# tomer-erez/Psychoacoustic-adverserial-attacks

Hardware: AMD Instinct MI355X
Metric: pgd_steps_per_sec (higher is better)
Workload: dtype bf16x3 (split-bf16 hi+lo, three MFMA passes, f32 accumulate: fp32-parity); 1 GPU; untargeted PGD, norm_type snr snr_db 40, Wav2Vec2-base (rule-generated weights), 32x10s 16 kHz clips per GPU, 150-token labels; global_batch=32, per_gpu_batch=32, samples_per_clip=160000, parallelism=dp1, hip_graph=True, hip_graph_replayed_steps=80

## Files before the change

psychoacoustic-adverserial-attacks_amd/csrc/gemm.hip:

```cpp
#include <algorithm>
#include <vector>

#include "gemm_dev.h"

namespace paa {

template <int ROWS, bool IS_A>
__device__ __forceinline__ void load_kc(const paa_gemm_desc& d, const float* __restrict__ base, int64_t ld, int r0,
                                        int k0, int rlim, float4 (&v)[ROWS / 32]) {
    const int tid = threadIdx.x;
    const int k = k0 + ((tid & 7) << 2);
    int64_t koff = k;
    int js = 0, kc = k;
    if (IS_A && d.a_kseg > 0) {
        js = k / d.a_kseg;
        kc = k - js * d.a_kseg;
        koff = (int64_t)js * d.a_kseg_stride + kc;
    }
#pragma unroll
    for (int i = 0; i < ROWS / 32; ++i) {
        const int r = r0 + (tid >> 3) + 32 * i;
        float4 x = make_float4(0.f, 0.f, 0.f, 0.f);
        bool ok = (r < rlim) && (k < d.K);
        const float* p;
// ... 536 lines not shown

static int g_ring_mode = 0;
struct GemmEnv { bool init = false, no_sq = false, no_r2 = false, kgroup = true, no_bil = false; };
static GemmEnv g_env;
static void gemm_env_refresh() {
#ifdef PAA_EXPERIMENTS
    auto on = [](const char* name, char v) { const char* e = getenv(name); return e && e[0] == v; };
    g_env.no_sq = on("PAA_NO_SQ", '1');
    g_env.no_r2 = on("PAA_NO_R2", '1');
    g_env.kgroup = !on("PAA_K_GROUP", '0');
    g_env.no_bil = on("PAA_NO_BIL", '1');
#endif
    g_env.init = true;
}
bool gemm_env_no_bil() {
    if (!g_env.init) gemm_env_refresh();
    return g_env.no_bil;
}
bool gemm_env_kgroup() {
    if (!g_env.init) gemm_env_refresh();
    return g_env.kgroup;
}

static int g_last_kind = EPK_GENERIC;
static int classify_epilogue(const paa_gemm_desc& d) {
#ifdef PAA_EXPERIMENTS
    { const char* e = getenv("PAA_NO_EPIK"); if (e && e[0] == '1') return EPK_GENERIC; }
#endif
    if (d.alpha != 1.f || d.accumulate || d.aux_bf16 || !d.precision) return EPK_GENERIC;
    const bool il = d.Cb_il && !d.Cb && !d.Cb_lo, planar = d.Cb && d.Cb_lo && !d.Cb_il, no_planes = !d.Cb && !d.Cb_lo && !d.Cb_il;
    const bool mask = d.row_period > 0;
    switch (d.act) {
        case PAA_ACT_GELU:
            return (d.bias && d.C_pre && d.aux_gate && il && !d.C && !d.aux && !d.residual && !d.res_ln_stats) ? EPK_GELU_FWD : EPK_GENERIC;
        case PAA_ACT_GELU_GRAD:
            if (!(d.aux && d.aux_gate && (il || planar) && !d.bias && !d.C && !d.C_pre && !d.residual && !d.res_ln_stats && !mask)) return EPK_GENERIC;
#ifdef PAA_EXPERIMENTS
            { const char* e = getenv("PAA_EPIK_AHEAD"); if (e && e[0] == '2') return EPK_GELU_GRAD_LA2; if (e && e[0] == '4') return EPK_GELU_GRAD_LA4; }
#endif
            return EPK_GELU_GRAD;
        case PAA_ACT_NONE:
            if (d.C_pre || d.aux || d.aux_gate || mask) return EPK_GENERIC;
            if (d.C && no_planes && d.residual) {
                if (d.res_ln_stats) return d.bias ? EPK_RESID_LN : EPK_GENERIC;
                return d.bias ? EPK_GENERIC : EPK_RESID;
            }
            if (!d.C && planar && !d.residual && !d.res_ln_stats) return EPK_PLANES;
            return EPK_GENERIC;
        default: return EPK_GENERIC;
    }
}

template <int BN, int PREC>
static void launch_gemm(const GemmArgs& g, dim3 grid, hipStream_t st) {
    const bool akc = g.d.a_kcontig != 0, bkc = g.d.b_kcontig != 0;
    if (akc && bkc) hipLaunchKernelGGL((k_gemm<BN, PREC, true, true>), grid, dim3(G_NT), 0, st, g);
    else if (akc && !bkc) hipLaunchKernelGGL((k_gemm<BN, PREC, true, false>), grid, dim3(G_NT), 0, st, g);
    else if (!akc && bkc) hipLaunchKernelGGL((k_gemm<BN, PREC, false, true>), grid, dim3(G_NT), 0, st, g);
    else hipLaunchKernelGGL((k_gemm<BN, PREC, false, false>), grid, dim3(G_NT), 0, st, g);
}

struct GemmProf {
    bool on = false;
    std::vector<hipEvent_t> ev;
    std::vector<double> flops, bytes;
    std::vector<int> variant;
    size_t n = 0, cap = 0;
};
static GemmProf g_prof;

paa_status gemm(const paa_gemm_desc& d, hipStream_t st) {
// ... 120 lines not shown
        d.ldb >= d.K && d.a_kseg_stride == d.lda) {
        const int taps = d.K / d.a_kseg;
        const int npl = d.precision ? 2 : 1;
        const int mi = (d.a_kseg == 48 && d.M > 128) ? 2 : 1;
        const size_t lds = 2 * (size_t)npl * ((size_t)(128 * mi + taps - 1) * (d.a_kseg + 8) + 64 * (size_t)(4 * d.a_kseg + 8));
        if (lds <= 150 * 1024) {
            dim3 wgrid(cdiv(d.M, 128 * mi), d.batch);
#define PAA_WIN(P, KS_, MI_, WV_)                                                                                            \
            {                                                                                                                \
                static bool attr = false;                                                                                    \
                if (!attr) { PAA_HIP(hipFuncSetAttribute(reinterpret_cast<const void*>(&k_gemm_win<P, KS_, MI_, WV_>), hipFuncAttributeMaxDynamicSharedMemorySize, 152 * 1024)); attr = true; } \
                hipLaunchKernelGGL((k_gemm_win<P, KS_, MI_, WV_>), wgrid, dim3(WV_ * 64), lds, st, g, taps);                 \
            }
            if (prof) { g_prof.variant[g_prof.n] = 40 + (d.precision ? 4 : 0); }
            if (d.a_kseg == 48) {
                if (mi == 2) { if (d.precision) PAA_WIN(1, 48, 1, 8) else PAA_WIN(0, 48, 2, 4) }
                else { if (d.precision) PAA_WIN(1, 48, 1, 4) else PAA_WIN(0, 48, 1, 4) }
            }
            else { if (d.precision) PAA_WIN(1, 64, 1, 4) else PAA_WIN(0, 64, 1, 4) }
#undef PAA_WIN
            if (prof) { (void)hipEventRecord(g_prof.ev[2 * g_prof.n + 1], st); ++g_prof.n; }
            PAA_LAUNCH_CHECK();
            return PAA_OK;
        }
    }
    if (ring) {
        if (prof) g_prof.variant[g_prof.n] = (ring_bm == 192 ? (ring_bn == 128 ? 60 : 52) : (ring_bn == 256 ? 56 : 48)) + (d.precision ? 1 : 0);
#ifdef PAA_EXPERIMENTS
        if (ring == 13) launch_bf<192, 128, 1, 2, true, false, true>(g, st);
        else
#endif
        if (ring >= 20) {
            g.kind = g_last_kind = classify_epilogue(d);
            int taken = 1 << EPK_GELU_FWD;
#ifdef PAA_EXPERIMENTS
            { const char* e = getenv("PAA_EPIK_MASK"); const int mask = e ? atoi(e) : 0; if (mask > 0) taken = mask; }
#endif
            if (!((taken >> g.kind) & 1)) g.kind = EPK_GENERIC;
            launch_ring2_cfg(ring, g, st);
        }
        else launch_ring_cfg(ring, g, st);
    } else if (d.operand_bf16) {
        const bool seg = d.a_kseg > 0 || (d.K & 63);
        if (narrow) {
            if (seg) { if (d.precision) launch_bf<128, 64, 1, 2, false, true>(g, st); else launch_bf<128, 64, 0, 2, false, true>(g, st); }
            else { if (d.precision) launch_bf<128, 64, 1, 2, false, false>(g, st); else launch_bf<128, 64, 0, 2, false, false>(g, st); }
        }
        else if (seg && vec && !d.precision) launch_bf<128, 128, 0, 2, true, true>(g, st);
        else if (seg) { if (d.precision) launch_bf<128, 128, 1, 2, false, true>(g, st); else launch_bf<128, 128, 0, 2, false, true>(g, st); }
        else if (tall) {
            if (d.precision) launch_bf<256, 128, 1, 4, true, false>(g, st);
            else if (bm192) launch_bf<192, 128, 0, 2, true, false>(g, st);
            else launch_bf<256, 128, 0, 2, true, false>(g, st);
        }
        else if (vec) { if (d.precision) launch_bf<128, 128, 1, 2, true, false>(g, st); else launch_bf<128, 128, 0, 2, true, false>(g, st); }
        else { if (d.precision) launch_bf<128, 128, 1, 2, false, false>(g, st); else launch_bf<128, 128, 0, 2, false, false>(g, st); }
    } else if (narrow) { if (d.precision) launch_gemm<64, 1>(g, grid, st); else launch_gemm<64, 0>(g, grid, st); }
    else { if (d.precision) launch_gemm<128, 1>(g, grid, st); else launch_gemm<128, 0>(g, grid, st); }
    if (prof) { (void)hipEventRecord(g_prof.ev[2 * g_prof.n + 1], st); ++g_prof.n; }
    PAA_LAUNCH_CHECK();
    return PAA_OK;
}

}

extern "C" paa_status paa_prof_enable(int max_launches) {
    using namespace paa;
// ... 44 lines not shown
```

psychoacoustic-adverserial-attacks_amd/csrc/gemm_dev.h:

```cpp
#pragma once
#include "gemm.h"
#include "paa_common.h"

namespace paa {

typedef short bf16x8 __attribute__((ext_vector_type(8)));
typedef float f32x16 __attribute__((ext_vector_type(16)));

constexpr int G_BM = 128, G_BK = 32, G_LD = 40 , G_NT = 256;


struct GemmArgs {
    paa_gemm_desc d;
    int tiles_m, tiles_n;
    int kind;
};

enum { EPK_GENERIC = 0, EPK_GELU_FWD = 1, EPK_GELU_GRAD = 2, EPK_RESID = 3, EPK_RESID_LN = 4, EPK_PLANES = 5,
       EPK_GELU_GRAD_LA2 = 6, EPK_GELU_GRAD_LA4 = 7, EPK_COUNT = 8 };
enum { EPI_NO = 0, EPI_YES = 1, EPI_RT = 2 };
template <int S>
__device__ __forceinline__ bool epi_on(bool rt) {
    if constexpr (S == EPI_RT) return rt;
    else return S == EPI_YES;
}
struct EpiGeneric {
    static constexpr int ACT = -1, BIAS = EPI_RT, C = EPI_RT, CPRE = EPI_RT, X16 = EPI_RT, GATE = EPI_RT, CIL = EPI_RT, CB = EPI_RT, CBLO = EPI_RT,
                         RES = EPI_RT, RLN = EPI_RT, PERIOD = EPI_RT, ACCUM = EPI_RT;
    static constexpr bool ALPHA1 = false;
    static constexpr int AHEAD = 1;
};
struct EpiGeluFwd {
    static constexpr int ACT = PAA_ACT_GELU, BIAS = EPI_YES, C = EPI_NO, CPRE = EPI_YES, X16 = EPI_NO, GATE = EPI_YES, CIL = EPI_YES, CB = EPI_NO, CBLO = EPI_NO,
                         RES = EPI_NO, RLN = EPI_NO, PERIOD = EPI_RT, ACCUM = EPI_NO;
    static constexpr bool ALPHA1 = true;
    static constexpr int AHEAD = 1;
};
struct EpiGeluGrad {
    static constexpr int ACT = PAA_ACT_GELU_GRAD, BIAS = EPI_NO, C = EPI_NO, CPRE = EPI_NO, X16 = EPI_NO, GATE = EPI_YES, CIL = EPI_RT, CB = EPI_YES, CBLO = EPI_YES,
                         RES = EPI_NO, RLN = EPI_NO, PERIOD = EPI_NO, ACCUM = EPI_NO;
    static constexpr bool ALPHA1 = true;
    static constexpr int AHEAD = 1;
};
template <int AH>
struct EpiGeluGradAhead : EpiGeluGrad {
    static constexpr int AHEAD = AH;
};
struct EpiResid {
    static constexpr int ACT = PAA_ACT_NONE, BIAS = EPI_NO, C = EPI_YES, CPRE = EPI_NO, X16 = EPI_NO, GATE = EPI_NO, CIL = EPI_NO, CB = EPI_NO, CBLO = EPI_NO,
                         RES = EPI_YES, RLN = EPI_NO, PERIOD = EPI_NO, ACCUM = EPI_NO;
    static constexpr bool ALPHA1 = true;
    static constexpr int AHEAD = 1;
};
struct EpiResidLn {
    static constexpr int ACT = PAA_ACT_NONE, BIAS = EPI_YES, C = EPI_YES, CPRE = EPI_NO, X16 = EPI_NO, GATE = EPI_NO, CIL = EPI_NO, CB = EPI_NO, CBLO = EPI_NO,
                         RES = EPI_YES, RLN = EPI_YES, PERIOD = EPI_NO, ACCUM = EPI_NO;
    static constexpr bool ALPHA1 = true;
    static constexpr int AHEAD = 1;
};
struct EpiPlanes {
    static constexpr int ACT = PAA_ACT_NONE, BIAS = EPI_RT, C = EPI_NO, CPRE = EPI_NO, X16 = EPI_NO, GATE = EPI_NO, CIL = EPI_NO, CB = EPI_YES, CBLO = EPI_YES,
                         RES = EPI_NO, RLN = EPI_NO, PERIOD = EPI_NO, ACCUM = EPI_NO;
    static constexpr bool ALPHA1 = true;
    static constexpr int AHEAD = 1;
};

template <typename K>
inline int blocks_per_cu(K kernel, int threads) {
    int per = 0;
    if (hipOccupancyMaxActiveBlocksPerMultiprocessor(&per, kernel, threads, 0) != hipSuccess) return 0;
    return per;
}

template <int NJ, int MI>
__device__ __forceinline__ void epilogue(const paa_gemm_desc& d, f32x16 (&acc)[MI][NJ], int mw, int nw, int z1, int z2) {
    const int64_t coff = z1 * d.c_s1 + z2 * d.c_s2 + (int64_t)mw * d.ldc + nw;
    float* __restrict__ C = d.C ? d.C + coff : nullptr;
    const bool x16 = d.aux_bf16 != 0;
    float* __restrict__ Cp = (d.C_pre && !x16) ? d.C_pre + coff : nullptr;
    unsigned short* __restrict__ Cp16 = (d.C_pre && x16) ? reinterpret_cast<unsigned short*>(d.C_pre) + coff : nullptr;
    unsigned short* __restrict__ Cb = d.Cb ? reinterpret_cast<unsigned short*>(d.Cb) + coff : nullptr;
    unsigned short* __restrict__ Cbl = d.Cb_lo ? reinterpret_cast<unsigned short*>(d.Cb_lo) + coff : nullptr;
    unsigned short* __restrict__ Cil = d.Cb_il ? reinterpret_cast<unsigned short*>(d.Cb_il) + 2 * (z1 * d.c_s1 + z2 * d.c_s2) : nullptr;
    const int64_t xoff = z1 * d.aux_s1 + z2 * d.aux_s2 + (int64_t)mw * d.ld_aux + nw;
    const float* __restrict__ aux = (d.aux && !x16) ? d.aux + xoff : nullptr;
    const unsigned short* __restrict__ aux16 = (d.aux && x16) ? reinterpret_cast<const unsigned short*>(d.aux) + xoff : nullptr;
    const float* __restrict__ res = d.residual ? d.residual + z1 * d.res_s1 + z2 * d.res_s2 + (int64_t)mw * d.ld_res + nw : nullptr;
    const float* __restrict__ bias = d.bias ? d.bias + z2 * d.bias_s2 + nw : nullptr;
    const int ldc = (int)d.ldc, ld_aux = (int)d.ld_aux, ld_res = (int)d.ld_res;
    const int period = d.row_period;
    const int mrem0 = period > 0 ? mw % period : 0;
    const int act = d.act;
    const float alpha = d.alpha;
#pragma unroll
    for (int i = 0; i < MI; ++i) {
        const int64_t ro = (int64_t)(i * 32) * ldc;
        float* __restrict__ Ci = C ? C + ro : nullptr;
// ... 55 lines not shown
                    Cbi[ci] = h;
                    if (Cbli) Cbli[ci] = bf16_bits(v - bf16_to_f32(h));
                }
                if (Cil) {
                    const int n = nw + dn;
                    const int64_t o = (int64_t)(mw + i * 32 + dm) * (2 * d.ldc) + ((n >> 5) << 6) + (n & 31);
                    const unsigned short h = bf16_bits(v);
                    Cil[o] = h;
                    Cil[o + 32] = bf16_bits(v - bf16_to_f32(h));
                }
            }
        }
    }
}

__device__ __forceinline__ float dpp_quad_xor1(float v) {
    return __int_as_float(__builtin_amdgcn_mov_dpp(__float_as_int(v), 0xB1, 0xF, 0xF, true));
}
__device__ __forceinline__ float dpp_quad_xor2(float v) {
    return __int_as_float(__builtin_amdgcn_mov_dpp(__float_as_int(v), 0x4E, 0xF, 0xF, true));
}
__device__ __forceinline__ void quad_transpose(float& x0, float& x1, float& x2, float& x3, bool o1, bool o2) {
    float s = dpp_quad_xor1(o1 ? x0 : x1);
    float t = dpp_quad_xor1(o1 ? x2 : x3);
    if (o1) { x0 = s; x2 = t; } else { x1 = s; x3 = t; }
    s = dpp_quad_xor2(o2 ? x0 : x2);
    t = dpp_quad_xor2(o2 ? x1 : x3);
    if (o2) { x0 = s; x1 = t; } else { x2 = s; x3 = t; }
}

__device__ __forceinline__ float mul_unfused(float a, float b) {
#pragma clang fp contract(off)
    return a * b;
}

template <int MI, bool FAST, typename T = EpiGeneric>
__device__ __forceinline__ void epilogue_vec(const paa_gemm_desc& d, f32x16 (&acc)[MI][2], int m0w, int n0w, int z1, int z2, int lane) {
    const int lr = lane & 31, lh = lane >> 5, qa = lr >> 2, qb = lr & 3;
    const bool o1 = qb & 1, o2 = qb & 2;
    const int col = n0w + 8 * qa;
    const int row0 = m0w + 4 * lh + qb;
    const bool col_ok = col < d.N;
    const int act = T::ACT < 0 ? d.act : T::ACT;
    const bool gg = act == PAA_ACT_GELU_GRAD;
    const int64_t cbase = z1 * d.c_s1 + z2 * d.c_s2;
    float* __restrict__ C = epi_on<T::C>(d.C != nullptr) ? d.C + cbase : nullptr;
    const bool has_c = T::C == EPI_RT ? C != nullptr : T::C == EPI_YES;
    const bool x16 = epi_on<T::X16>(d.aux_bf16 != 0);
    const bool gate = epi_on<T::GATE>(d.aux_gate != 0);
    float* __restrict__ Cp = (epi_on<T::CPRE>(d.C_pre != nullptr) && !x16) ? d.C_pre + cbase : nullptr;
    unsigned short* __restrict__ Cp16 = (epi_on<T::CPRE>(d.C_pre != nullptr) && x16) ? reinterpret_cast<unsigned short*>(d.C_pre) + cbase : nullptr;
    constexpr bool PRE_RT = T::CPRE == EPI_RT || T::X16 == EPI_RT;
    const bool has_cp = PRE_RT ? Cp != nullptr : (T::CPRE == EPI_YES && T::X16 == EPI_NO);
    const bool has_cp16 = PRE_RT ? Cp16 != nullptr : (T::CPRE == EPI_YES && T::X16 == EPI_YES);
    unsigned short* __restrict__ Cb = epi_on<T::CB>(d.Cb != nullptr) ? reinterpret_cast<unsigned short*>(d.Cb) + cbase : nullptr;
    unsigned short* __restrict__ Cbl = epi_on<T::CBLO>(d.Cb_lo != nullptr) ? reinterpret_cast<unsigned short*>(d.Cb_lo) + cbase : nullptr;
    const bool cil = epi_on<T::CIL>(d.Cb_il != nullptr);
    if (cil) { Cb = reinterpret_cast<unsigned short*>(d.Cb_il) + 2 * cbase; Cbl = Cb + 32; }
    const bool has_cb = (T::CIL == EPI_YES || T::CB == EPI_YES) ? true : (T::CIL == EPI_NO && T::CB == EPI_NO) ? false : Cb != nullptr;
    const bool has_cbl = (T::CIL == EPI_YES || T::CBLO == EPI_YES) ? true : (T::CIL == EPI_NO && T::CBLO == EPI_NO) ? false : Cbl != nullptr;
    const bool ex16 = gg && x16;
    const float* __restrict__ ex = gg ? (ex16 ? nullptr : d.aux + z1 * d.aux_s1 + z2 * d.aux_s2)
                                      : (epi_on<T::RES>(d.residual != nullptr) ? d.residual + z1 * d.res_s1 + z2 * d.res_s2 : nullptr);
    const unsigned short* __restrict__ exh = ex16 ? reinterpret_cast<const unsigned short*>(d.aux) + z1 * d.aux_s1 + z2 * d.aux_s2 : nullptr;
    constexpr bool EX_RT = T::ACT < 0 || T::X16 == EPI_RT || T::RES == EPI_RT;
    const bool has_ex = EX_RT ? ex != nullptr : (gg ? !ex16 : T::RES == EPI_YES);
    const bool has_exh = EX_RT ? exh != nullptr : ex16;
    const unsigned ldc = (unsigned)d.ldc, ldx = (unsigned)(gg ? d.ld_aux : d.ld_res);
    const unsigned co = (unsigned)row0 * ldc + (unsigned)col;
    const unsigned cob = cil ? (unsigned)row0 * 2u * ldc + (((unsigned)col >> 5) << 6) + ((unsigned)col & 31u) : co;
    const unsigned ldcb = cil ? 2u * ldc : ldc;
    const unsigned xo = (unsigned)row0 * ldx + (unsigned)col;
    float bv[8];
#pragma unroll
    for (int k = 0; k < 8; ++k) bv[k] = 0.f;
    if (epi_on<T::BIAS>(d.bias != nullptr) && col_ok) {
        const float* bp = d.bias + z2 * d.bias_s2;
        const float4 b0 = *reinterpret_cast<const float4*>(bp + (unsigned)col);
        const float4 b1 = *reinterpret_cast<const float4*>(bp + (unsigned)col + 4u);
        bv[0] = b0.x; bv[1] = b0.y; bv[2] = b0.z; bv[3] = b0.w; bv[4] = b1.x; bv[5] = b1.y; bv[6] = b1.z; bv[7] = b1.w;
    }
    const bool rln = epi_on<T::RLN>(d.res_ln_stats != nullptr) && !gg && has_ex;
    constexpr bool RLN_HELD = MI < 4;
    float lg[8], lb[8];
#pragma unroll
    for (int k = 0; k < 8; ++k) { lg[k] = 1.f; lb[k] = 0.f; }
    if (RLN_HELD && rln && col_ok) {
        const float4 g0 = *reinterpret_cast<const float4*>(d.res_ln_g + (unsigned)col), g1 = *reinterpret_cast<const float4*>(d.res_ln_g + (unsigned)col + 4u);
        const float4 b0 = *reinterpret_cast<const float4*>(d.res_ln_b + (unsigned)col), b1 = *reinterpret_cast<const float4*>(d.res_ln_b + (unsigned)col + 4u);
        lg[0] = g0.x; lg[1] = g0.y; lg[2] = g0.z; lg[3] = g0.w; lg[4] = g1.x; lg[5] = g1.y; lg[6] = g1.z; lg[7] = g1.w;
        lb[0] = b0.x; lb[1] = b0.y; lb[2] = b0.z; lb[3] = b0.w; lb[4] = b1.x; lb[5] = b1.y; lb[6] = b1.z; lb[7] = b1.w;
    }
    const int period = T::PERIOD == EPI_NO ? 0 : d.row_period;
    const int mrem0 = period > 0 ? row0 % period : 0;
    const float alpha = T::ALPHA1 ? 1.f : d.alpha;
    const bool accum = epi_on<T::ACCUM>(d.accumulate != 0);
    constexpr int NG = 4 * MI;
    constexpr int AH = T::AHEAD < NG ? T::AHEAD : NG - 1, NX = AH + 1;
    uint4 xv[NX][2];
#pragma unroll
    for (int u = 0; u < NX; ++u) { xv[u][0] = make_uint4(0u, 0u, 0u, 0u); xv[u][1] = xv[u][0]; }
    auto fetch = [&](int grp, uint4 (&v2)[2]) {
        const int dm = (grp >> 2) * 32 + (grp & 3) * 8;
        if (col_ok && row0 + dm < d.M) {
            const unsigned o = xo + (unsigned)dm * ldx;
            if (has_ex) {
                v2[0] = *reinterpret_cast<const uint4*>(ex + o);
                v2[1] = *reinterpret_cast<const uint4*>(ex + o + 4u);
            } else if (has_exh) {
                v2[0] = *reinterpret_cast<const uint4*>(exh + o);
            }
        }
    };
#pragma unroll
    for (int a = 0; a < AH; ++a) fetch(a, xv[a]);
#pragma unroll
    for (int grp = 0; grp < NG; ++grp) {
        const int i = grp >> 2, gq = grp & 3, u = grp % NX;
        if (grp + AH < NG) fetch(grp + AH, xv[(grp + AH) % NX]);
        const int dm = i * 32 + gq * 8;
        const bool live = col_ok && row0 + dm < d.M;
        bool dead = false;
        if (period > 0) {
            int rem = mrem0 + dm;
            if (rem >= period) rem = (period >= 256) ? rem - period : rem % period;
            dead = rem >= d.row_valid;
        }
        const unsigned ci = co + (unsigned)dm * ldc;
        float2 rst = make_float2(0.f, 1.f);
        if (rln && live) rst = *reinterpret_cast<const float2*>(d.res_ln_stats + 2 * (size_t)(row0 + dm));
        unsigned hp[4], lp[4], pp[4];
#pragma unroll
        for (int j = 0; j < 2; ++j) {
            float x[4] = {acc[i][j][4 * gq], acc[i][j][4 * gq + 1], acc[i][j][4 * gq + 2], acc[i][j][4 * gq + 3]};
            quad_transpose(x[0], x[1], x[2], x[3], o1, o2);
            float e4[4];
            if (ex16) {
                const unsigned w0 = j ? xv[u][0].z : xv[u][0].x, w1 = j ? xv[u][0].w : xv[u][0].y;
                e4[0] = __uint_as_float(w0 << 16); e4[1] = __uint_as_float(w0 & 0xFFFF0000u);
                e4[2] = __uint_as_float(w1 << 16); e4[3] = __uint_as_float(w1 & 0xFFFF0000u);
            } else {
                e4[0] = __uint_as_float(xv[u][j].x); e4[1] = __uint_as_float(xv[u][j].y);
                e4[2] = __uint_as_float(xv[u][j].z); e4[3] = __uint_as_float(xv[u][j].w);
            }
            if (rln) {
                if constexpr (RLN_HELD) {
#pragma unroll
                    for (int k = 0; k < 4; ++k) e4[k] = (e4[k] - rst.x) * rst.y * lg[4 * j + k] + lb[4 * j + k];
                } else {
                    float4 g4 = make_float4(1.f, 1.f, 1.f, 1.f), b4 = make_float4(0.f, 0.f, 0.f, 0.f);
                    if (col_ok) {
                        g4 = *reinterpret_cast<const float4*>(d.res_ln_g + (unsigned)col + 4u * j);
                        b4 = *reinterpret_cast<const float4*>(d.res_ln_b + (unsigned)col + 4u * j);
                    }
                    e4[0] = (e4[0] - rst.x) * rst.y * g4.x + b4.x; e4[1] = (e4[1] - rst.x) * rst.y * g4.y + b4.y;
                    e4[2] = (e4[2] - rst.x) * rst.y * g4.z + b4.z; e4[3] = (e4[3] - rst.x) * rst.y * g4.w + b4.w;
                }
            }
#pragma unroll
            for (int k = 0; k < 4; ++k) x[k] = x[k] * alpha + bv[4 * j + k];
            if (act == PAA_ACT_GELU) {
                float kp[4];
                if (FAST) {
// ... 18 lines not shown
                }
                if (has_ex) {
#pragma unroll
                    for (int k = 0; k < 4; ++k) x[k] += e4[k];
                }
            } else if (gg) {
#pragma unroll
                for (int k = 0; k < 4; ++k) x[k] = mul_unfused(x[k], gate ? e4[k] : (FAST ? gelu_grad_fast(e4[k]) : gelu_grad_f(e4[k])));
            } else if (has_ex) {
#pragma unroll
                for (int k = 0; k < 4; ++k) x[k] += e4[k];
            }
            if (dead) {
#pragma unroll
                for (int k = 0; k < 4; ++k) x[k] = 0.f;
            }
            if (has_c && live) {
                if (accum) {
                    const float4 c0 = *reinterpret_cast<const float4*>(C + ci + 4u * j);
                    x[0] += c0.x; x[1] += c0.y; x[2] += c0.z; x[3] += c0.w;
                }
                *reinterpret_cast<float4*>(C + ci + 4u * j) = make_float4(x[0], x[1], x[2], x[3]);
            }
            if (has_cb) {
                const unsigned h01 = bf16_pack2(x[0], x[1]), h23 = bf16_pack2(x[2], x[3]);
                hp[2 * j] = h01; hp[2 * j + 1] = h23;
                if (has_cbl) {
                    lp[2 * j] = bf16_pack2(x[0] - __uint_as_float(h01 << 16), x[1] - __uint_as_float(h01 & 0xFFFF0000u));
                    lp[2 * j + 1] = bf16_pack2(x[2] - __uint_as_float(h23 << 16), x[3] - __uint_as_float(h23 & 0xFFFF0000u));
                }
            }
            __builtin_amdgcn_sched_barrier(0);
        }
        if (has_cp16 && live && act == PAA_ACT_GELU) *reinterpret_cast<uint4*>(Cp16 + ci) = make_uint4(pp[0], pp[1], pp[2], pp[3]);
        if (has_cb && live) {
            const unsigned cb = cob + (unsigned)dm * ldcb;
            *reinterpret_cast<uint4*>(Cb + cb) = make_uint4(hp[0], hp[1], hp[2], hp[3]);
            if (has_cbl) *reinterpret_cast<uint4*>(Cbl + cb) = make_uint4(lp[0], lp[1], lp[2], lp[3]);
        }
    }
}

}
```

psychoacoustic-adverserial-attacks_amd/csrc/gemm_ring2.hip:

```cpp
#include <stdlib.h>

#include <algorithm>

#include "gemm_dev.h"

namespace paa {

bool gemm_env_no_bil();

namespace {

#if defined(PAA_R2_DEFER) && !defined(PAA_EXPERIMENTS)
#error "PAA_R2_DEFER is a diagnostic build: add -DPAA_EXPERIMENTS"
#endif
#ifndef PAA_R2_DEFER
#define PAA_R2_DEFER 1
#endif
#if (defined(PAA_R2_A_AUX) || defined(PAA_R2_B_AUX)) && !defined(PAA_EXPERIMENTS)
#error "PAA_R2_A_AUX / PAA_R2_B_AUX are diagnostic builds: add -DPAA_EXPERIMENTS"
#endif
#ifndef PAA_R2_A_AUX
#define PAA_R2_A_AUX 0
#endif
#ifndef PAA_R2_PRIO_BALANCE
#define PAA_R2_PRIO_BALANCE 1
#endif
#ifndef PAA_R2_B_AUX
#define PAA_R2_B_AUX 0
#endif
typedef __attribute__((address_space(1))) const void* gas_ptr2;
typedef __attribute__((address_space(3))) void* las_ptr2;
template <int N>
__device__ __forceinline__ void wait_vmcnt2() { asm volatile("s_waitcnt vmcnt(%0)" ::"n"(N) : "memory"); }

#if defined(PAA_R2_STAMP) && !defined(PAA_EXPERIMENTS)
#error "PAA_R2_STAMP is a diagnostic build: add -DPAA_EXPERIMENTS"
#endif
#ifdef PAA_R2_STAMP
__device__ long long g_r2_stamp[8 * 16 * 6];
#define R2_NOW() ((long long)__builtin_amdgcn_s_memtime())
#endif

template <int BM, int BN, int BK, int PREC, int WR, int WC, bool BIL = false, bool AIL = false, typename EPI = EpiGeneric>
__global__ __launch_bounds__(WR * WC * 64, 2) void k_gemm_ring2(GemmArgs g) {
    constexpr int NW = WR * WC;
    constexpr int NPL = PREC ? 2 : 1;
    constexpr int RB = BK * 2;
    constexpr int CPR = RB / 16;
    constexpr int RPI = 1024 / RB;
    constexpr int RBR = 256 / RB;
    constexpr int NSTA = 3, NSTB = 2;
    static_assert(!BIL || (PREC == 1 && BK == 32), "interleaved planes: split mode, one 32-element K group per slab");
    constexpr int RBB = BIL ? 128 : RB, CPRB = RBB / 16, RPIB = 1024 / RBB, RBRB = 256 / RBB;
    static_assert(!AIL || (PREC == 1 && BK == 32 && BM % (8 * WR * WC) == 0), "interleaved A planes: split mode, one 32-element K group per slab");
    constexpr int RBA = AIL ? 128 : RB, CPRA = RBA / 16, RPIA = 1024 / RBA, RBRA = 256 / RBA;
    constexpr int ASZ = NPL * BM * RB, BSZ = NPL * BN * RB;
    constexpr int GA = ASZ / 1024 / NW, GB = BSZ / 1024 / NW;
    constexpr int MI = BM / WR / 32, NJ = BN / WC / 32, KS = BK / 16;
    constexpr bool DEFER = PAA_R2_DEFER && PREC;
    static_assert(NJ == 2, "vector epilogue: 64 columns per wave");
    static_assert((NPL * BM) % (RPI * NW) == 0 && (NPL * BN) % (RPI * NW) == 0 && BM % RPI == 0 && BN % RPI == 0 && BSZ % (1024 * NW) == 0, "a DMA wave-instruction must not straddle planes");
    static_assert(NSTA * ASZ + NSTB * BSZ <= 160 * 1024 && GA + GB < 32, "rings do not fit");
    __shared__ __attribute__((aligned(1024))) unsigned char smem[NSTA * ASZ + NSTB * BSZ];
    unsigned char* const smA = smem;
    unsigned char* const smB = smem + NSTA * ASZ;

// ... 8 lines not shown
    if ((int)blockIdx.x >= total) return;

    struct Tile { int m0, n0, z1, z2; };
    auto decode = [&](int t) {
        Tile c;
        const int z = t / nwg, orig = t - z * nwg;
        const int q = nwg >> 3, r8 = nwg & 7, xcd = orig & 7;
        const int id = (xcd < r8 ? xcd * (q + 1) : r8 * (q + 1) + (xcd - r8) * q) + (orig >> 3);
        const int tm = id / g.tiles_n, tn = id - tm * g.tiles_n;
        c.m0 = tm * BM; c.n0 = tn * BN;
        c.z1 = z / d.batch2; c.z2 = z - c.z1 * d.batch2;
        return c;
    };
    const int kg_spt = (d.k_group > 0 && d.k_group % BK == 0 && d.K % d.k_group == 0 && d.K > d.k_group) ? d.k_group / BK : 0;
    const int kg_taps = kg_spt ? d.K / d.k_group : 1;

    struct Cursor { int t, k, tap, c, slab, slot; };
    auto advance = [&](Cursor& u, int nslots) {
        u.slot = u.slot + 1 == nslots ? 0 : u.slot + 1;
        if (kg_spt) {
            if (++u.tap == kg_taps) { u.tap = 0; ++u.c; }
            u.slab = u.tap * kg_spt + u.c;
        } else {
            ++u.slab;
        }
        if (++u.k == nk) {
            u.k = 0; u.tap = 0; u.c = 0; u.slab = 0;
            u.t += gridDim.x;
            return true;
        }
        return false;
    };
    Cursor ca{(int)blockIdx.x, 0, 0, 0, 0, 0}, cb = ca;
    const unsigned short* srcA[GA];
    const unsigned short* srcB[GB];
    auto set_srcA = [&](int t) {
        const Tile c = decode(t);
        const int64_t aoff = c.z1 * d.a_s1 + c.z2 * d.a_s2;
        int lane_o;
        asm volatile("v_mbcnt_lo_u32_b32 %0, -1, 0\n\tv_mbcnt_hi_u32_b32 %0, -1, %0" : "=v"(lane_o));
#pragma unroll
        for (int i = 0; i < GA; ++i) {
            if constexpr (AIL) {
                const int rr = (i * NW + wave) * RPIA + lane_o / CPRA;
                const int ch = (lane_o % CPRA) ^ ((rr / RBRA) & (CPRA - 1));
                srcA[i] = reinterpret_cast<const unsigned short*>(d.A_il) + 2 * aoff + (int64_t)min(c.m0 + rr, d.M - 1) * (2 * d.lda) + ch * 8;
            } else {
                const int r = (i * NW + wave) * RPI + lane_o / CPR;
                const int pl = r / BM, rr = r - pl * BM;
                const int ch = (lane_o % CPR) ^ ((rr / RBR) & (CPR - 1));
                const unsigned short* A = reinterpret_cast<const unsigned short*>(pl ? d.A_lo : (const void*)d.A) + aoff;
                srcA[i] = A + (int64_t)min(c.m0 + rr, d.M - 1) * d.lda + ch * 8;
            }
        }
    };
    auto set_srcB = [&](int t) {
        const Tile c = decode(t);
        const int64_t boff = c.z1 * d.b_s1 + c.z2 * d.b_s2;
        int lane_o;
        asm volatile("v_mbcnt_lo_u32_b32 %0, -1, 0\n\tv_mbcnt_hi_u32_b32 %0, -1, %0" : "=v"(lane_o));
#pragma unroll
        for (int i = 0; i < GB; ++i) {
            const int r = (i * NW + wave) * RPIB + lane_o / CPRB;
            const int pl = BIL ? 0 : r / BN, p = r - pl * BN;
            const int ch = (lane_o % CPRB) ^ ((p / RBRB) & (CPRB - 1));
            const int nl = (p & ~63) + 8 * ((p & 31) >> 2) + 4 * ((p >> 5) & 1) + (p & 3);
            if constexpr (BIL) {
                srcB[i] = reinterpret_cast<const unsigned short*>(d.B_il) + 2 * boff + (int64_t)min(c.n0 + nl, d.N - 1) * (2 * d.ldb) + ch * 8;
            } else {
                const unsigned short* B = reinterpret_cast<const unsigned short*>(pl ? d.B_lo : (const void*)d.B) + boff;
                srcB[i] = B + (int64_t)min(c.n0 + nl, d.N - 1) * d.ldb + ch * 8;
            }
        }
    };
    auto issueA = [&]() {
        if (ca.t >= total) return false;
        unsigned char* st = smA + ca.slot * ASZ;
#pragma unroll
        for (int i = 0; i < GA; ++i)
            __builtin_amdgcn_global_load_lds((gas_ptr2)(srcA[i] + (int64_t)ca.slab * (AIL ? 2 * BK : BK)), (las_ptr2)(st + (i * NW + wave) * 1024), 16, 0, PAA_R2_A_AUX);
        if (advance(ca, NSTA) && ca.t < total) set_srcA(ca.t);
        return true;
    };
    auto issueB = [&]() {
        if (cb.t >= total) return;
        unsigned char* st = smB + cb.slot * BSZ;
#pragma unroll
        for (int i = 0; i < GB; ++i)
            __builtin_amdgcn_global_load_lds((gas_ptr2)(srcB[i] + (int64_t)cb.slab * (BIL ? 2 * BK : BK)), (las_ptr2)(st + (i * NW + wave) * 1024), 16, 0, PAA_R2_B_AUX);
        if (advance(cb, NSTB) && cb.t < total) set_srcB(cb.t);
    };
    set_srcA(ca.t);
    set_srcB(cb.t);
    issueB();
    issueA();
    bool ahead = issueA();
    if (ahead) wait_vmcnt2<GA>(); else wait_vmcnt2<0>();
    __builtin_amdgcn_sched_barrier(0);
    __builtin_amdgcn_s_barrier();
    __builtin_amdgcn_sched_barrier(0);

    const int sw = (lr / RBR) & (CPR - 1);
    int offk[KS];
#pragma unroll
    for (int ks = 0; ks < KS; ++ks) offk[ks] = ((2 * ks + lh) ^ sw) << 4;
    const int arow = (wr * (BM / WR) + lr) * RBA, brow = (wc * (BN / WC) + lr) * RBB;
    constexpr int ALO = BM * RB, BLO = BN * RB;
    const int swa = (lr / RBRA) & (CPRA - 1);
    int offah[KS], offal[KS];
#pragma unroll
    for (int ks = 0; ks < KS; ++ks) {
        offah[ks] = AIL ? (((2 * ks + lh) ^ swa) << 4) : offk[ks];
        offal[ks] = AIL ? (((4 + 2 * ks + lh) ^ swa) << 4) : ALO + offk[ks];
    }
    const int swb = (lr / RBRB) & (CPRB - 1);
    int offbh[KS], offbl[KS];
#pragma unroll
    for (int ks = 0; ks < KS; ++ks) {
        offbh[ks] = BIL ? (((2 * ks + lh) ^ swb) << 4) : offk[ks];
        offbl[ks] = BIL ? (((4 + 2 * ks + lh) ^ swb) << 4) : BLO + offk[ks];
    }

// ... 117 lines not shown
                    }
                }
            if (!DEFER || last) {
                if (ahead) wait_vmcnt2<GA>(); else wait_vmcnt2<0>();
                __builtin_amdgcn_sched_barrier(0);
                __builtin_amdgcn_s_barrier();
                __builtin_amdgcn_sched_barrier(0);
            }
        }
#ifdef PAA_R2_STAMP
        const long long st_t1 = R2_NOW();
#endif
        epilogue_vec<MI, true, EPI>(d, acc, cur.m0 + wr * (BM / WR), cur.n0 + wc * (BN / WC), cur.z1, cur.z2, lane);
#ifdef PAA_R2_STAMP
        if (blockIdx.x == 0 && lane == 0 && st_tile < 16) {
            long long* o = g_r2_stamp + (wave * 16 + st_tile) * 6;
            o[0] = nk; o[1] = st_t1 - st_t0; o[2] = st_vm; o[3] = st_bar; o[4] = R2_NOW() - st_t1; o[5] = st_t0;
        }
        ++st_tile;
#endif
    }
}

template <int BM, int BN, int BK, int PREC, int WR, int WC, bool BIL, bool AIL, typename EPI = EpiGeneric>
void launch_ring2_il(const GemmArgs& g, hipStream_t st) {
    static const int per_cu = blocks_per_cu(k_gemm_ring2<BM, BN, BK, PREC, WR, WC, BIL, AIL, EPI>, WR * WC * 64);
    const int resident = per_cu * device_cus();
    const int total = g.tiles_m * g.tiles_n * g.d.batch;
    const int blocks = resident > 0 ? std::min(total, resident) : total;
    hipLaunchKernelGGL((k_gemm_ring2<BM, BN, BK, PREC, WR, WC, BIL, AIL, EPI>), dim3(blocks), dim3(WR * WC * 64), 0, st, g);
}
template <int BM, int BN, int BK, int WR, int WC, bool AIL>
void launch_ring2_kind(const GemmArgs& g, hipStream_t st) {
    if (g.kind == EPK_GELU_FWD) { launch_ring2_il<BM, BN, BK, 1, WR, WC, true, AIL, EpiGeluFwd>(g, st); return; }
#ifdef PAA_EXPERIMENTS
    switch (g.kind) {
        case EPK_GELU_GRAD: launch_ring2_il<BM, BN, BK, 1, WR, WC, true, AIL, EpiGeluGrad>(g, st); return;
        case EPK_GELU_GRAD_LA2: launch_ring2_il<BM, BN, BK, 1, WR, WC, true, AIL, EpiGeluGradAhead<2>>(g, st); return;
        case EPK_GELU_GRAD_LA4: launch_ring2_il<BM, BN, BK, 1, WR, WC, true, AIL, EpiGeluGradAhead<4>>(g, st); return;
        default: break;
    }
    if constexpr (BM == 192) {
        switch (g.kind) {
            case EPK_RESID: launch_ring2_il<BM, BN, BK, 1, WR, WC, true, AIL, EpiResid>(g, st); return;
            case EPK_RESID_LN: launch_ring2_il<BM, BN, BK, 1, WR, WC, true, AIL, EpiResidLn>(g, st); return;
            case EPK_PLANES: launch_ring2_il<BM, BN, BK, 1, WR, WC, true, AIL, EpiPlanes>(g, st); return;
            default: break;
        }
    }
#endif
    launch_ring2_il<BM, BN, BK, 1, WR, WC, true, AIL>(g, st);
}
template <int BM, int BN, int BK, int PREC, int WR, int WC>
void launch_ring2(const GemmArgs& g, hipStream_t st) {
    if constexpr (PREC == 1) {
        const bool bil = g.d.B_il && g.d.b_s1 == 0 && g.d.b_s2 == 0 && !gemm_env_no_bil();
        if (g.d.A_il) {
            if (bil) launch_ring2_kind<BM, BN, BK, WR, WC, true>(g, st);
            else launch_ring2_il<BM, BN, BK, PREC, WR, WC, false, true>(g, st);
            return;
        }
        if (bil) { launch_ring2_kind<BM, BN, BK, WR, WC, false>(g, st); return; }
    }
    launch_ring2_il<BM, BN, BK, PREC, WR, WC, false, false>(g, st);
}

}

#ifdef PAA_R2_STAMP
}
extern "C" int paa_debug_r2_stamps(long long* host) {
    if (hipDeviceSynchronize() != hipSuccess) return 1;
    if (hipMemcpyFromSymbol(host, HIP_SYMBOL(paa::g_r2_stamp), sizeof(long long) * 8 * 16 * 6) != hipSuccess) return 1;
    static long long zeros[8 * 16 * 6];
    return hipMemcpyToSymbol(HIP_SYMBOL(paa::g_r2_stamp), zeros, sizeof(zeros)) == hipSuccess ? 0 : 1;
}
namespace paa {
#endif

void launch_ring2_cfg(int cfg, const GemmArgs& g, hipStream_t st) {
    switch (cfg) {
        case 20: launch_ring2<256, 256, 32, 1, 2, 4>(g, st); break;
        case 21: launch_ring2<256, 256, 64, 0, 2, 4>(g, st); break;
// ... 8 lines not shown
```

Before: 28.84 steps/s (one step = PGD step on 32 x 10 s clips; counted over all ranks).

## Ship specialized GELU-grad and planes epilogues; switch ring loads to buffer DMA

The default set of specialized epilogues in the ring2 GEMM grows: GELU-grad and planar-output kernels now run by default, and the GELU-forward path also covers calls without bias. The epilogue prefetch now clamps rows instead of branching, can prefetch layer-norm stats ahead, and adds register-landing fences plus an early-settle option for GELU-grad. The global-to-LDS ring loads move from per-lane 64-bit pointers to buffer_load_lds with a scalar resource and small integer offsets, which cuts VGPR use and address arithmetic. These are several independent changes, and they bring risk around offset overflow and out-of-bounds behaviour.

After: 29.69 steps/s (one step = PGD step on 32 x 10 s clips; counted over all ranks), median of 6. 1.03x the previous value.

```diff
diff --git a/psychoacoustic-adverserial-attacks_amd/csrc/gemm.hip b/psychoacoustic-adverserial-attacks_amd/csrc/gemm.hip
--- a/psychoacoustic-adverserial-attacks_amd/csrc/gemm.hip
+++ b/psychoacoustic-adverserial-attacks_amd/csrc/gemm.hip
@@ -592,11 +592,12 @@
     const bool mask = d.row_period > 0;
     switch (d.act) {
         case PAA_ACT_GELU:
-            return (d.bias && d.C_pre && d.aux_gate && il && !d.C && !d.aux && !d.residual && !d.res_ln_stats) ? EPK_GELU_FWD : EPK_GENERIC;
+            return (d.C_pre && d.aux_gate && il && !d.C && !d.aux && !d.residual && !d.res_ln_stats) ? EPK_GELU_FWD : EPK_GENERIC;
         case PAA_ACT_GELU_GRAD:
             if (!(d.aux && d.aux_gate && (il || planar) && !d.bias && !d.C && !d.C_pre && !d.residual && !d.res_ln_stats && !mask)) return EPK_GENERIC;
 #ifdef PAA_EXPERIMENTS
-            { const char* e = getenv("PAA_EPIK_AHEAD"); if (e && e[0] == '2') return EPK_GELU_GRAD_LA2; if (e && e[0] == '4') return EPK_GELU_GRAD_LA4; }
+            { const char* e = getenv("PAA_EPIK_AHEAD"); if (e && e[0] == '2') return EPK_GELU_GRAD_LA2; if (e && e[0] == '4') return EPK_GELU_GRAD_LA4;
+              if (e && e[0] == '1') return EPK_GELU_GRAD_LA1; }
 #endif
             return EPK_GELU_GRAD;
         case PAA_ACT_NONE:
@@ -783,7 +784,7 @@
 #endif
         if (ring >= 20) {
             g.kind = g_last_kind = classify_epilogue(d);
-            int taken = 1 << EPK_GELU_FWD;
+            int taken = EPK_SHIPPED;
 #ifdef PAA_EXPERIMENTS
             { const char* e = getenv("PAA_EPIK_MASK"); const int mask = e ? atoi(e) : 0; if (mask > 0) taken = mask; }
 #endif
diff --git a/psychoacoustic-adverserial-attacks_amd/csrc/gemm_dev.h b/psychoacoustic-adverserial-attacks_amd/csrc/gemm_dev.h
--- a/psychoacoustic-adverserial-attacks_amd/csrc/gemm_dev.h
+++ b/psychoacoustic-adverserial-attacks_amd/csrc/gemm_dev.h
@@ -17,7 +17,8 @@
 };
 
 enum { EPK_GENERIC = 0, EPK_GELU_FWD = 1, EPK_GELU_GRAD = 2, EPK_RESID = 3, EPK_RESID_LN = 4, EPK_PLANES = 5,
-       EPK_GELU_GRAD_LA2 = 6, EPK_GELU_GRAD_LA4 = 7, EPK_COUNT = 8 };
+       EPK_GELU_GRAD_LA2 = 6, EPK_GELU_GRAD_LA4 = 7, EPK_GELU_GRAD_LA1 = 8, EPK_COUNT = 9 };
+constexpr int EPK_SHIPPED = (1 << EPK_GELU_FWD) | (1 << EPK_GELU_GRAD) | (1 << EPK_PLANES);
 enum { EPI_NO = 0, EPI_YES = 1, EPI_RT = 2 };
 template <int S>
 __device__ __forceinline__ bool epi_on(bool rt) {
@@ -29,40 +30,47 @@
                          RES = EPI_RT, RLN = EPI_RT, PERIOD = EPI_RT, ACCUM = EPI_RT;
     static constexpr bool ALPHA1 = false;
     static constexpr int AHEAD = 1;
+    static constexpr bool SETTLE_EARLY = false;
 };
 struct EpiGeluFwd {
-    static constexpr int ACT = PAA_ACT_GELU, BIAS = EPI_YES, C = EPI_NO, CPRE = EPI_YES, X16 = EPI_NO, GATE = EPI_YES, CIL = EPI_YES, CB = EPI_NO, CBLO = EPI_NO,
+    static constexpr int ACT = PAA_ACT_GELU, BIAS = EPI_RT, C = EPI_NO, CPRE = EPI_YES, X16 = EPI_NO, GATE = EPI_YES, CIL = EPI_YES, CB = EPI_NO, CBLO = EPI_NO,
                          RES = EPI_NO, RLN = EPI_NO, PERIOD = EPI_RT, ACCUM = EPI_NO;
     static constexpr bool ALPHA1 = true;
     static constexpr int AHEAD = 1;
+    static constexpr bool SETTLE_EARLY = false;
 };
 struct EpiGeluGrad {
     static constexpr int ACT = PAA_ACT_GELU_GRAD, BIAS = EPI_NO, C = EPI_NO, CPRE = EPI_NO, X16 = EPI_NO, GATE = EPI_YES, CIL = EPI_RT, CB = EPI_YES, CBLO = EPI_YES,
                          RES = EPI_NO, RLN = EPI_NO, PERIOD = EPI_NO, ACCUM = EPI_NO;
     static constexpr bool ALPHA1 = true;
     static constexpr int AHEAD = 1;
+    static constexpr bool SETTLE_EARLY = true;
 };
 template <int AH>
 struct EpiGeluGradAhead : EpiGeluGrad {
     static constexpr int AHEAD = AH;
+    static constexpr bool SETTLE_EARLY = false;
 };
 struct EpiResid {
     static constexpr int ACT = PAA_ACT_NONE, BIAS = EPI_NO, C = EPI_YES, CPRE = EPI_NO, X16 = EPI_NO, GATE = EPI_NO, CIL = EPI_NO, CB = EPI_NO, CBLO = EPI_NO,
                          RES = EPI_YES, RLN = EPI_NO, PERIOD = EPI_NO, ACCUM = EPI_NO;
     static constexpr bool ALPHA1 = true;
     static constexpr int AHEAD = 1;
+    static constexpr bool SETTLE_EARLY = false;
 };
 struct EpiResidLn {
     static constexpr int ACT = PAA_ACT_NONE, BIAS = EPI_YES, C = EPI_YES, CPRE = EPI_NO, X16 = EPI_NO, GATE = EPI_NO, CIL = EPI_NO, CB = EPI_NO, CBLO = EPI_NO,
                          RES = EPI_YES, RLN = EPI_YES, PERIOD = EPI_NO, ACCUM = EPI_NO;
     static constexpr bool ALPHA1 = true;
     static constexpr int AHEAD = 1;
+    static constexpr bool SETTLE_EARLY = false;
 };
 struct EpiPlanes {
     static constexpr int ACT = PAA_ACT_NONE, BIAS = EPI_RT, C = EPI_NO, CPRE = EPI_NO, X16 = EPI_NO, GATE = EPI_NO, CIL = EPI_NO, CB = EPI_YES, CBLO = EPI_YES,
                          RES = EPI_NO, RLN = EPI_NO, PERIOD = EPI_NO, ACCUM = EPI_NO;
     static constexpr bool ALPHA1 = true;
     static constexpr int AHEAD = 1;
+    static constexpr bool SETTLE_EARLY = false;
 };
 
 template <typename K>
@@ -184,6 +192,13 @@
 __device__ __forceinline__ float mul_unfused(float a, float b) {
 #pragma clang fp contract(off)
     return a * b;
+}
+
+__device__ __forceinline__ void epi_landed(const uint4& v) { asm volatile("" ::"v"(v.x), "v"(v.y), "v"(v.z), "v"(v.w)); }
+template <int N>
+__device__ __forceinline__ void epi_landed(const float (&v)[N]) {
+#pragma unroll
+    for (int k = 0; k < N; ++k) asm volatile("" ::"v"(v[k]));
 }
 
 template <int MI, bool FAST, typename T = EpiGeneric>
@@ -222,7 +237,6 @@
     const unsigned co = (unsigned)row0 * ldc + (unsigned)col;
     const unsigned cob = cil ? (unsigned)row0 * 2u * ldc + (((unsigned)col >> 5) << 6) + ((unsigned)col & 31u) : co;
     const unsigned ldcb = cil ? 2u * ldc : ldc;
-    const unsigned xo = (unsigned)row0 * ldx + (unsigned)col;
     float bv[8];
 #pragma unroll
     for (int k = 0; k < 8; ++k) bv[k] = 0.f;
@@ -250,26 +264,38 @@
     constexpr int NG = 4 * MI;
     constexpr int AH = T::AHEAD < NG ? T::AHEAD : NG - 1, NX = AH + 1;
     uint4 xv[NX][2];
-#pragma unroll
-    for (int u = 0; u < NX; ++u) { xv[u][0] = make_uint4(0u, 0u, 0u, 0u); xv[u][1] = xv[u][0]; }
-    auto fetch = [&](int grp, uint4 (&v2)[2]) {
-        const int dm = (grp >> 2) * 32 + (grp & 3) * 8;
-        if (col_ok && row0 + dm < d.M) {
-            const unsigned o = xo + (unsigned)dm * ldx;
-            if (has_ex) {
-                v2[0] = *reinterpret_cast<const uint4*>(ex + o);
-                v2[1] = *reinterpret_cast<const uint4*>(ex + o + 4u);
-            } else if (has_exh) {
-                v2[0] = *reinterpret_cast<const uint4*>(exh + o);
-            }
+    constexpr bool RS_AHEAD = T::RLN == EPI_YES;
+    float rsv[NX][2];
+    constexpr bool EARLY = T::SETTLE_EARLY && AH == 1 && T::ACT == PAA_ACT_GELU_GRAD && T::X16 != EPI_RT && T::C == EPI_NO && T::CPRE == EPI_NO;
+    constexpr bool EX_ANY = EX_RT || T::ACT == PAA_ACT_GELU_GRAD || T::RES == EPI_YES;
+#pragma unroll
+    for (int u = 0; u < NX; ++u) { xv[u][0] = make_uint4(0u, 0u, 0u, 0u); xv[u][1] = xv[u][0]; rsv[u][0] = 0.f; rsv[u][1] = 1.f; }
+    auto fetch = [&](int grp, uint4 (&v2)[2], float (&r2)[2]) {
+        const unsigned rowc = (unsigned)min(row0 + (grp >> 2) * 32 + (grp & 3) * 8, d.M - 1);
+        if (RS_AHEAD && rln) {
+            const float2 st = *reinterpret_cast<const float2*>(d.res_ln_stats + 2 * (size_t)rowc);
+            r2[0] = st.x; r2[1] = st.y;
+        }
+        const unsigned o = rowc * ldx + (col_ok ? (unsigned)col : 0u);
+        if (has_ex) {
+            v2[0] = *reinterpret_cast<const uint4*>(ex + o);
+            v2[1] = *reinterpret_cast<const uint4*>(ex + o + 4u);
+        } else if (has_exh) {
+            v2[0] = *reinterpret_cast<const uint4*>(exh + o);
         }
     };
 #pragma unroll
-    for (int a = 0; a < AH; ++a) fetch(a, xv[a]);
+    for (int a = 0; a < AH; ++a) fetch(a, xv[a], rsv[a]);
 #pragma unroll
     for (int grp = 0; grp < NG; ++grp) {
         const int i = grp >> 2, gq = grp & 3, u = grp % NX;
-        if (grp + AH < NG) fetch(grp + AH, xv[(grp + AH) % NX]);
+        if (grp + AH < NG) fetch(grp + AH, xv[(grp + AH) % NX], rsv[(grp + AH) % NX]);
+        if (grp == 0) {
+            if constexpr (T::BIAS != EPI_NO) epi_landed(bv);
+            if constexpr (RLN_HELD && T::RLN != EPI_NO) { epi_landed(lg); epi_landed(lb); }
+        }
+        if constexpr (EX_ANY) { epi_landed(xv[u][0]); epi_landed(xv[u][1]); }
+        if constexpr (RS_AHEAD) epi_landed(rsv[u]);
         const int dm = i * 32 + gq * 8;
         const bool live = col_ok && row0 + dm < d.M;
         bool dead = false;
@@ -279,8 +305,8 @@
             dead = rem >= d.row_valid;
         }
         const unsigned ci = co + (unsigned)dm * ldc;
-        float2 rst = make_float2(0.f, 1.f);
-        if (rln && live) rst = *reinterpret_cast<const float2*>(d.res_ln_stats + 2 * (size_t)(row0 + dm));
+        float2 rst = make_float2(rsv[u][0], rsv[u][1]);
+        if (!RS_AHEAD && rln && live) rst = *reinterpret_cast<const float2*>(d.res_ln_stats + 2 * (size_t)(row0 + dm));
         unsigned hp[4], lp[4], pp[4];
 #pragma unroll
         for (int j = 0; j < 2; ++j) {
@@ -365,6 +391,9 @@
             }
             __builtin_amdgcn_sched_barrier(0);
         }
+        if constexpr (EARLY) {
+            if (grp + 1 < NG) { epi_landed(xv[(grp + 1) % NX][0]); epi_landed(xv[(grp + 1) % NX][1]); }
+        }
         if (has_cp16 && live && act == PAA_ACT_GELU) *reinterpret_cast<uint4*>(Cp16 + ci) = make_uint4(pp[0], pp[1], pp[2], pp[3]);
         if (has_cb && live) {
             const unsigned cb = cob + (unsigned)dm * ldcb;
diff --git a/psychoacoustic-adverserial-attacks_amd/csrc/gemm_ring2.hip b/psychoacoustic-adverserial-attacks_amd/csrc/gemm_ring2.hip
--- a/psychoacoustic-adverserial-attacks_amd/csrc/gemm_ring2.hip
+++ b/psychoacoustic-adverserial-attacks_amd/csrc/gemm_ring2.hip
@@ -28,10 +28,22 @@
 #ifndef PAA_R2_B_AUX
 #define PAA_R2_B_AUX 0
 #endif
-typedef __attribute__((address_space(1))) const void* gas_ptr2;
 typedef __attribute__((address_space(3))) void* las_ptr2;
 template <int N>
-__device__ __forceinline__ void wait_vmcnt2() { asm volatile("s_waitcnt vmcnt(%0)" ::"n"(N) : "memory"); }
+__device__ __forceinline__ void wait_vmcnt2() {
+    static_assert(N >= 0 && N < 64, "vmcnt is six bits");
+    __builtin_amdgcn_s_waitcnt((N & 15) | ((N >> 4) << 14) | 0x0F70);
+}
+template <int AUX>
+__device__ __forceinline__ void ring2_dma(const void* base, las_ptr2 dst, int voff, int soff) {
+#if defined(__HIP_DEVICE_COMPILE__)
+    const unsigned long long b = (unsigned long long)base;
+    const unsigned long long u = ((unsigned long long)(unsigned)__builtin_amdgcn_readfirstlane((int)(b >> 32)) << 32) |
+                                 (unsigned)__builtin_amdgcn_readfirstlane((int)(unsigned)b);
+    __builtin_amdgcn_raw_ptr_buffer_load_lds(__builtin_amdgcn_make_buffer_rsrc((void*)u, 0, -1, 0x00020000), dst, 16, voff,
+                                             __builtin_amdgcn_readfirstlane(soff), 0, AUX);
+#endif
+}
 
 #if defined(PAA_R2_STAMP) && !defined(PAA_EXPERIMENTS)
 #error "PAA_R2_STAMP is a diagnostic build: add -DPAA_EXPERIMENTS"
@@ -106,25 +118,31 @@
         return false;
     };
     Cursor ca{(int)blockIdx.x, 0, 0, 0, 0, 0}, cb = ca;
-    const unsigned short* srcA[GA];
-    const unsigned short* srcB[GB];
+    const unsigned short *rsA[NPL], *rsB[NPL];
+    int offA[GA], offB[GB];
     auto set_srcA = [&](int t) {
         const Tile c = decode(t);
         const int64_t aoff = c.z1 * d.a_s1 + c.z2 * d.a_s2;
         int lane_o;
         asm volatile("v_mbcnt_lo_u32_b32 %0, -1, 0\n\tv_mbcnt_hi_u32_b32 %0, -1, %0" : "=v"(lane_o));
+        const int mlast = d.M - 1 - c.m0;
+        if constexpr (AIL) {
+            rsA[0] = reinterpret_cast<const unsigned short*>(d.A_il) + 2 * aoff + (int64_t)c.m0 * (2 * d.lda);
+        } else {
+            rsA[0] = reinterpret_cast<const unsigned short*>(d.A) + aoff + (int64_t)c.m0 * d.lda;
+            if constexpr (NPL == 2) rsA[1] = reinterpret_cast<const unsigned short*>(d.A_lo) + aoff + (int64_t)c.m0 * d.lda;
+        }
 #pragma unroll
         for (int i = 0; i < GA; ++i) {
             if constexpr (AIL) {
                 const int rr = (i * NW + wave) * RPIA + lane_o / CPRA;
                 const int ch = (lane_o % CPRA) ^ ((rr / RBRA) & (CPRA - 1));
-                srcA[i] = reinterpret_cast<const unsigned short*>(d.A_il) + 2 * aoff + (int64_t)min(c.m0 + rr, d.M - 1) * (2 * d.lda) + ch * 8;
+                offA[i] = min(rr, mlast) * (int)(4 * d.lda) + ch * 16;
             } else {
                 const int r = (i * NW + wave) * RPI + lane_o / CPR;
-                const int pl = r / BM, rr = r - pl * BM;
+                const int rr = r % BM;
                 const int ch = (lane_o % CPR) ^ ((rr / RBR) & (CPR - 1));
-                const unsigned short* A = reinterpret_cast<const unsigned short*>(pl ? d.A_lo : (const void*)d.A) + aoff;
-                srcA[i] = A + (int64_t)min(c.m0 + rr, d.M - 1) * d.lda + ch * 8;
+                offA[i] = min(rr, mlast) * (int)(2 * d.lda) + ch * 16;
             }
         }
     };
@@ -133,35 +151,41 @@
         const int64_t boff = c.z1 * d.b_s1 + c.z2 * d.b_s2;
         int lane_o;
         asm volatile("v_mbcnt_lo_u32_b32 %0, -1, 0\n\tv_mbcnt_hi_u32_b32 %0, -1, %0" : "=v"(lane_o));
+        const int nlast = d.N - 1 - c.n0;
+        if constexpr (BIL) {
+            rsB[0] = reinterpret_cast<const unsigned short*>(d.B_il) + 2 * boff + (int64_t)c.n0 * (2 * d.ldb);
+        } else {
+            rsB[0] = reinterpret_cast<const unsigned short*>(d.B) + boff + (int64_t)c.n0 * d.ldb;
+            if constexpr (NPL == 2) rsB[1] = reinterpret_cast<const unsigned short*>(d.B_lo) + boff + (int64_t)c.n0 * d.ldb;
+        }
 #pragma unroll
         for (int i = 0; i < GB; ++i) {
             const int r = (i * NW + wave) * RPIB + lane_o / CPRB;
-            const int pl = BIL ? 0 : r / BN, p = r - pl * BN;
+            const int p = BIL ? r : r % BN;
             const int ch = (lane_o % CPRB) ^ ((p / RBRB) & (CPRB - 1));
             const int nl = (p & ~63) + 8 * ((p & 31) >> 2) + 4 * ((p >> 5) & 1) + (p & 3);
-            if constexpr (BIL) {
-                srcB[i] = reinterpret_cast<const unsigned short*>(d.B_il) + 2 * boff + (int64_t)min(c.n0 + nl, d.N - 1) * (2 * d.ldb) + ch * 8;
-            } else {
-                const unsigned short* B = reinterpret_cast<const unsigned short*>(pl ? d.B_lo : (const void*)d.B) + boff;
-                srcB[i] = B + (int64_t)min(c.n0 + nl, d.N - 1) * d.ldb + ch * 8;
-            }
-        }
-    };
+            offB[i] = min(nl, nlast) * (int)((BIL ? 4 : 2) * d.ldb) + ch * 16;
+        }
+    };
+    auto planeA = [&](int i) { return AIL ? 0 : ((i * NW + wave) * RPI) / BM; };
+    auto planeB = [&](int i) { return BIL ? 0 : ((i * NW + wave) * RPIB) / BN; };
     auto issueA = [&]() {
         if (ca.t >= total) return false;
         unsigned char* st = smA + ca.slot * ASZ;
+        const int so = ca.slab * ((AIL ? 2 * BK : BK) * 2);
 #pragma unroll
         for (int i = 0; i < GA; ++i)
-            __builtin_amdgcn_global_load_lds((gas_ptr2)(srcA[i] + (int64_t)ca.slab * (AIL ? 2 * BK : BK)), (las_ptr2)(st + (i * NW + wave) * 1024), 16, 0, PAA_R2_A_AUX);
+            ring2_dma<PAA_R2_A_AUX>(NPL == 2 && planeA(i) ? rsA[NPL - 1] : rsA[0], (las_ptr2)(st + (i * NW + wave) * 1024), offA[i], so);
         if (advance(ca, NSTA) && ca.t < total) set_srcA(ca.t);
         return true;
     };
     auto issueB = [&]() {
         if (cb.t >= total) return;
         unsigned char* st = smB + cb.slot * BSZ;
+        const int so = cb.slab * ((BIL ? 2 * BK : BK) * 2);
 #pragma unroll
         for (int i = 0; i < GB; ++i)
-            __builtin_amdgcn_global_load_lds((gas_ptr2)(srcB[i] + (int64_t)cb.slab * (BIL ? 2 * BK : BK)), (las_ptr2)(st + (i * NW + wave) * 1024), 16, 0, PAA_R2_B_AUX);
+            ring2_dma<PAA_R2_B_AUX>(NPL == 2 && planeB(i) ? rsB[NPL - 1] : rsB[0], (las_ptr2)(st + (i * NW + wave) * 1024), offB[i], so);
         if (advance(cb, NSTB) && cb.t < total) set_srcB(cb.t);
     };
     set_srcA(ca.t);
@@ -345,23 +369,26 @@
 }
 template <int BM, int BN, int BK, int WR, int WC, bool AIL>
 void launch_ring2_kind(const GemmArgs& g, hipStream_t st) {
-    if (g.kind == EPK_GELU_FWD) { launch_ring2_il<BM, BN, BK, 1, WR, WC, true, AIL, EpiGeluFwd>(g, st); return; }
+    switch (g.kind) {
+        case EPK_GELU_FWD: launch_ring2_il<BM, BN, BK, 1, WR, WC, true, AIL, EpiGeluFwd>(g, st); return;
+        case EPK_GELU_GRAD: launch_ring2_il<BM, BN, BK, 1, WR, WC, true, AIL, EpiGeluGrad>(g, st); return;
 #ifdef PAA_EXPERIMENTS
-    switch (g.kind) {
-        case EPK_GELU_GRAD: launch_ring2_il<BM, BN, BK, 1, WR, WC, true, AIL, EpiGeluGrad>(g, st); return;
         case EPK_GELU_GRAD_LA2: launch_ring2_il<BM, BN, BK, 1, WR, WC, true, AIL, EpiGeluGradAhead<2>>(g, st); return;
         case EPK_GELU_GRAD_LA4: launch_ring2_il<BM, BN, BK, 1, WR, WC, true, AIL, EpiGeluGradAhead<4>>(g, st); return;
+        case EPK_GELU_GRAD_LA1: launch_ring2_il<BM, BN, BK, 1, WR, WC, true, AIL, EpiGeluGradAhead<1>>(g, st); return;
+#endif
         default: break;
     }
     if constexpr (BM == 192) {
         switch (g.kind) {
+            case EPK_PLANES: launch_ring2_il<BM, BN, BK, 1, WR, WC, true, AIL, EpiPlanes>(g, st); return;
+#ifdef PAA_EXPERIMENTS
             case EPK_RESID: launch_ring2_il<BM, BN, BK, 1, WR, WC, true, AIL, EpiResid>(g, st); return;
             case EPK_RESID_LN: launch_ring2_il<BM, BN, BK, 1, WR, WC, true, AIL, EpiResidLn>(g, st); return;
-            case EPK_PLANES: launch_ring2_il<BM, BN, BK, 1, WR, WC, true, AIL, EpiPlanes>(g, st); return;
+#endif
             default: break;
         }
     }
-#endif
     launch_ring2_il<BM, BN, BK, 1, WR, WC, true, AIL>(g, st);
 }
 template <int BM, int BN, int BK, int PREC, int WR, int WC>
```
